# lux-liang/Robust-Audio-Deepfake-Evolution

Measured on AMD Instinct MI355X. Metric: Phase-6 train throughput (utterances/sec), DualStreamSEMamba + LoRA + RawBoost/codec + FGM, higher is better.
Workload: dtype fp16; 1 GPU; Phase6_Proposed.conf train step on ASVspoof19-LA-shaped utterances; micro_batch=8, accumulation=4, global_batch=32, seq_len=64600, parallelism=dp1, fgm=True, mixup=True, rawboost_algo=5, lora_mode=reference, hip_graphs=True, window_batched_clean_passes=True

## Files before the change

### include/radhip.h

```cpp
#ifndef RADHIP_H
#define RADHIP_H

#include <stdint.h>

#ifdef __cplusplus
extern "C" {
#endif

#define RDX_OK 0
#define RDX_EINVAL (-1)
#define RDX_EUNSUPPORTED (-2)

typedef enum { RDX_F32 = 0, RDX_BF16 = 1 } rdx_dtype;

const char* rdx_version(void);
const char* rdx_strerror(int code);

int rdx_sincconv_absmaxpool_fwd(const float* x, int64_t batch, int64_t len, const float* filters,
                                int channels, int ksize, int mask_lo, int mask_hi, float* out,
                                void* stream);
int rdx_sincconv_absmaxpool_fwd_devmask(const float* x, int64_t batch, int64_t len,
                                        const float* filters, int channels, int ksize,
                                        const int32_t* mask_dev, int mask_stride, float* out,
                                        void* stream);
// ... 315 lines not shown
int rdx_adamw_many_max(void);
int rdx_adamw_many(int n, float* const* params, float* const* grads, float* const* exp_avg, float* const* exp_avg_sq,
                   const float* const* step, const int64_t* numel, double lr, double beta1, double beta2,
                   double weight_decay, double eps, const float* grad_scale, const float* found_inf, void* stream);

int rdx_timestamp_acc(int64_t* acc, int sign, void* stream);
int rdx_wallclock_khz(int device);

int rdx_gemm_bf16_strided(const void* A, int64_t lda, int64_t sA, const void* B, int64_t ldb, void* C, int64_t ldc,
                          int64_t crow, int batch, int M, int N, int K, const void* bias, void* stream);

int rdx_fe_conv0(const float* x, int64_t batch, int64_t len, const float* w, const float* bias, const float* gamma,
                 const float* beta, float eps, int ksize, int stride, void* out, void* stream);
int rdx_fe_ln_gelu(void* io, int64_t rows, const float* gamma, const float* beta, float eps, float* out32,
                   void* stream);

int rdx_sconv_fwd(const void* x, const void* w, void* y, void* y2, const float* bn, int N, int H, int W, int ci,
                  int co, int kh, int ph, void* stream);
int rdx_sconv_fwd_res(const void* x, const void* w, void* y, const void* res, int N, int H, int W, int ci, int co,
                      int kh, int ph, void* stream);
int rdx_sconv_dgrad_bnselu(const void* dy, const void* w, const void* c, void* dc, const float* bn, float* sums,
                           int N, int H, int W, int ci, int co, int kh, int ph, void* stream);
int rdx_sconv_fwd_pool(const void* x, const void* w, const void* idn, const float* bias, void* y, uint8_t* arg, int N,
                       int H, int W, int ci, int co, void* stream);
int rdx_sconv_fwd_res_pool(const void* x, const void* w, void* y, const void* dp, const uint8_t* arg, float* dbias,
                           int N, int H, int W, int ci, int co, int kh, int ph, void* stream);
int rdx_sconv_dgrad_bnselu_pool(const void* dp, const uint8_t* arg, const void* w, const void* c, void* dc,
                                const float* bn, float* sums, int N, int H, int W, int ci, int co, int kh, int ph,
                                void* stream);
int rdx_sconv_dgrad_pool(const void* dp, const uint8_t* arg, const void* w, void* dx, int N, int H, int W, int ci,
                         int co, int kh, int ph, void* stream);
int rdx_sconv_wgrad_pool(const void* x, const void* dp, const uint8_t* arg, float* dw, float* part, int N, int H,
                         int W, int ci, int co, int kh, int ph, void* stream);
int rdx_sconv_wgrad_nblk(int N, int Ho, int W);
int rdx_sconv_wgrad(const void* x, const void* dy, float* dw, float* part, int N, int H, int W, int ci, int co,
                    int kh, int ph, void* stream);
int rdx_se_fwd(const void* x, const void* w1, const void* w2, void* y, void* m, void* h, void* s, int B, int T, int C,
               int R, void* stream);
int64_t rdx_se_bwd_part_floats(int B, int C, int R);
int rdx_se_bwd(const void* dy, const void* x, const void* w1, const void* w2, const void* m, const void* h, const void* s,
               void* dx, float* part, float* dw1, float* dw2, int B, int T, int C, int R, void* stream);
int rdx_attn_pool_fwd(const void* f, const void* w, const void* bias, void* feat, float* a, int B, int T, int C,
                      void* stream);
int rdx_attn_pool_bwd(const void* f, const void* w, const float* a, const void* dfeat, void* df, float* part, float* dw,
                      float* db, int B, int T, int C, void* stream);
int rdx_upcat_fwd(const void* fw, const void* fs, void* out, int B, int T1, int T2, int C, void* stream);
int rdx_upcat_bwd(const void* dout, void* dfs, int B, int T1, int T2, int C, void* stream);
int rdx_sconv_wprep_many(int n, const float* const* src, void* const* wf, void* const* wd, const int* co,
                         const int* ci, const int* kh, void* stream);

#ifdef __cplusplus
}
#endif
#endif
```

### robust-audio-deepfake-evolution_amd/csrc/sconv.hip

```cpp
#include <climits>
#include <initializer_list>

#include "common.h"

namespace rdx {

typedef __attribute__((ext_vector_type(16))) float sf32x16;
typedef __attribute__((ext_vector_type(2))) unsigned int v2u32;

constexpr int SC_T = 256;
constexpr int SC_P = 128;
constexpr int SC_PW = SC_P + 2;

__device__ __forceinline__ sf32x16 sc_mfma(hx8 a, hx8 b, sf32x16 c) {
  return mfma32x32x16(a, b, c);
}
__device__ __forceinline__ uint32_t sc_pack2(float a, float b) {
  hst x = f2h(a), y = f2h(b);
  return (uint32_t)(*reinterpret_cast<uint16_t*>(&x)) | ((uint32_t)(*reinterpret_cast<uint16_t*>(&y)) << 16);
}
__device__ __forceinline__ float sc_selu(float u) {
  return 1.0507009873554805f * (u > 0.f ? u : 1.6732632423543772f * (__expf(u) - 1.0f));
}

template <int C>
__device__ __forceinline__ int sc_off(int row, int ch) {
  constexpr int NCH = C / 8;
  return row * (C * 2) + 16 * (ch ^ (row & (NCH - 1)));
}

struct SConvArgs {
  const hst* x;
  const hst* w;
  hst* y;
  hst* y2;
  const float* bn;
  const hst* c;
  float* sums;
  const hst* res;
  const uint8_t* xarg;
  const uint8_t* rarg;
  uint8_t* parg;
  int N, H, W, Ho, ph;
  int rows_per;
};

constexpr uint32_t SC_OOB = 0x80000000u;

__device__ __forceinline__ __amdgpu_buffer_rsrc_t sc_rsrc(const void* p, int64_t bytes) {
  return __builtin_amdgcn_make_buffer_rsrc(const_cast<void*>(p), 0, (int)bytes, 0x00020000);
}

template <int CI, int PW = SC_PW>
__device__ __forceinline__ void sc_load_row(uint4* regs, __amdgpu_buffer_rsrc_t rs, int hi, int H, int W, int p0) {
  constexpr int XCH = CI / 8, NV = (PW * XCH + SC_T - 1) / SC_T;
  const bool rok = hi >= 0 && hi < H;
#pragma unroll
  for (int j = 0; j < NV; ++j) {
    const int i = threadIdx.x + SC_T * j;
    const int ch = i % XCH, pp = i / XCH, wi = p0 - 1 + pp;
    const bool ok = rok && pp < PW && wi >= 0 && wi < W;
    const uint32_t off = ok ? (uint32_t)(((hi * W + wi) * CI + ch * 8) * 2) : SC_OOB;
    regs[j] = __builtin_bit_cast(uint4, __builtin_amdgcn_raw_buffer_load_b128(rs, off, 0, 0));
  }
}
template <int CI, int PW = SC_PW>
__device__ __forceinline__ void sc_store_row(char* slot, const uint4* regs) {
  constexpr int XCH = CI / 8, NV = (PW * XCH + SC_T - 1) / SC_T;
#pragma unroll
  for (int j = 0; j < NV; ++j) {
    const int i = threadIdx.x + SC_T * j;
    if (i < PW * XCH) *reinterpret_cast<uint4*>(slot + sc_off<CI>(i / XCH, i % XCH)) = regs[j];
  }
}

__device__ __forceinline__ uint32_t sc_exp2(uint32_t d, uint32_t ab, uint32_t j) {
  return d & (((ab & 0xffu) == j ? 0xffffu : 0u) | (((ab >> 8) & 0xffu) == j ? 0xffff0000u : 0u));
}
__device__ __forceinline__ uint4 sc_expand(uint4 d, uint2 ab, uint32_t j) {
  return make_uint4(sc_exp2(d.x, ab.x, j), sc_exp2(d.y, ab.x >> 16, j), sc_exp2(d.z, ab.y, j),
                    sc_exp2(d.w, ab.y >> 16, j));
}

template <int CI>
__device__ __forceinline__ void sc_load_row_exp(uint4* regs, uint2* aregs, __amdgpu_buffer_rsrc_t rs,
                                                __amdgpu_buffer_rsrc_t ra, int hi, int H, int Wo, int p0) {
  constexpr int XCH = CI / 8, NV = (SC_PW * XCH + SC_T - 1) / SC_T;
  const bool rok = hi >= 0 && hi < H;
#pragma unroll
  for (int j = 0; j < NV; ++j) {
    const int i = threadIdx.x + SC_T * j;
    const int ch = i % XCH, pp = i / XCH, wi = p0 - 1 + pp;
    const int wo = wi / 3;
    const bool ok = rok && pp < SC_PW && wi >= 0 && wo < Wo;
    const uint32_t e = (uint32_t)((hi * Wo + wo) * CI + ch * 8);
    regs[j] = __builtin_bit_cast(uint4, __builtin_amdgcn_raw_buffer_load_b128(rs, ok ? e * 2 : SC_OOB, 0, 0));
    aregs[j] = __builtin_bit_cast(uint2, __builtin_amdgcn_raw_buffer_load_b64(ra, ok ? e : SC_OOB, 0, 0));
  }
}
template <int CI>
__device__ __forceinline__ void sc_store_row_exp(char* slot, const uint4* regs, const uint2* aregs, int p0) {
  constexpr int XCH = CI / 8, NV = (SC_PW * XCH + SC_T - 1) / SC_T;
#pragma unroll
  for (int j = 0; j < NV; ++j) {
// ... 242 lines not shown
    __syncthreads();
  }
  if constexpr (NSUM > 0) {
#pragma unroll
    for (int q = 0; q < NSUM; ++q)
#pragma unroll
      for (int t = 0; t < NT; ++t)
#pragma unroll
        for (int g = 0; g < 4; ++g)
#pragma unroll
          for (int e = 0; e < 4; ++e) {
            float x = bsum[q][t][g][e];
#pragma unroll
            for (int o = 1; o < 32; o <<= 1) x += __shfl_xor(x, o, 64);
            bsum[q][t][g][e] = x;
          }
    float* red = reinterpret_cast<float*>(sc_lds);
    if (r == 0) {
#pragma unroll
      for (int q = 0; q < NSUM; ++q)
#pragma unroll
        for (int t = 0; t < NT; ++t)
#pragma unroll
          for (int g = 0; g < 4; ++g)
#pragma unroll
            for (int e = 0; e < 4; ++e) red[(wv * NSUM + q) * CO + t * 32 + 8 * g + 4 * h + e] = bsum[q][t][g][e];
    }
    __syncthreads();
    for (int i = tid; i < NSUM * CO; i += SC_T)
      atomicAdd(&a.sums[i], (red[i] + red[NSUM * CO + i]) + (red[2 * NSUM * CO + i] + red[3 * NSUM * CO + i]));
  }
}

struct SWgradArgs {
  const hst* x;
  const hst* dy;
  const uint8_t* arg;
  float* part;
  int N, H, W, Ho, ph;
  int64_t units;
  int strips, nz, rows_per;
};


template <int C>
__device__ __forceinline__ int sc_img(int row, int ch) {
  return (C * 16) * (row >> 3) + 512 * (ch >> 2) + 64 * (row & 7) + 16 * ((ch & 3) ^ ((row >> 2) & 3));
}
template <int C>
__device__ __forceinline__ hx8 sc_read_tr(const char* img, int r0, int c0, int s, int lane) {
  const int g = lane >> 4, i = lane & 15;
  const int row = r0 + 16 * s + 4 * (g >> 1) + (i >> 2);
  const int col = c0 + 16 * (g & 1) + 4 * (i & 3);
  const int sub = 2 * (col & 7);
  const hx4v lo = ds_tr4((img + sc_img<C>(row, col >> 3) + sub));
  const hx4v hi = ds_tr4((img + sc_img<C>(row + 8, col >> 3) + sub));
  hx8 r;
#pragma unroll
  for (int j = 0; j < 4; ++j) {
    r[j] = lo[j];
    r[4 + j] = hi[j];
  }
  return r;
}

constexpr int SC_XR = 136;
// ... 134 lines not shown
  sconv_wgrad_body<CI, CO, KH, true>(a);
}

constexpr int SC_RS = 16;
__global__ void sconv_wgrad_reduce1_kernel(const float* __restrict__ part, int nblk, int64_t n, float* __restrict__ part2) {
  const int64_t i = (int64_t)blockIdx.x * blockDim.x + threadIdx.x;
  if (i >= n) return;
  const int per = (nblk + SC_RS - 1) / SC_RS, b0 = blockIdx.y * per, b1 = min(nblk, b0 + per);
  float s[8] = {0.f, 0.f, 0.f, 0.f, 0.f, 0.f, 0.f, 0.f};
  int b = b0;
  for (; b + 8 <= b1; b += 8) {
#pragma unroll
    for (int k = 0; k < 8; ++k) s[k] += part[(int64_t)(b + k) * n + i];
  }
  for (; b < b1; ++b) s[0] += part[(int64_t)b * n + i];
  part2[(int64_t)blockIdx.y * n + i] = ((s[0] + s[1]) + (s[2] + s[3])) + ((s[4] + s[5]) + (s[6] + s[7]));
}
__global__ void sconv_wgrad_reduce2_kernel(const float* __restrict__ part2, int64_t n, float* __restrict__ dw) {
  const int64_t i = (int64_t)blockIdx.x * blockDim.x + threadIdx.x;
  if (i >= n) return;
  float s = 0.f;
#pragma unroll
  for (int z = 0; z < SC_RS; ++z) s += part2[(int64_t)z * n + i];
  dw[i] = s;
}

static int sc_per_cu(size_t smem) {
  const int n = (int)((160 * 1024) / smem);
  return n < 1 ? 1 : (n > 4 ? 4 : n);
}

static size_t sc_wgrad_smem(int ci, int co, int kh) { return (2 * (size_t)SC_P * co + (size_t)(kh + 1) * SC_XR * ci) * 2; }

template <int CI, int CO, int KH, bool kBnBwd = false, bool kPool = false, bool kExpIn = false, bool kExpRes = false>
static int sconv_fwd_launch(const SConvArgs& a, hipStream_t st) {
  if ((int64_t)a.H * a.W * CI * 2 >= (int64_t)SC_OOB - 4096 || (int64_t)a.Ho * a.W * CO * 2 >= (int64_t)SC_OOB - 4096)
    return RDX_EUNSUPPORTED;
  if ((kPool || kExpIn || kExpRes) && a.W < 3) return RDX_EUNSUPPORTED;
  const size_t smem = (size_t)(KH + 1) * (kPool ? SC_PPW : SC_PW) * CI * 2 + (size_t)KH * 3 * CO * CI * 2 +
                      5 * CO * sizeof(float);
  const int strips = kPool ? (a.W / 3 * 3 + SC_PP - 1) / SC_PP : (a.W + SC_P - 1) / SC_P;
  const int64_t slots = 256 * (int64_t)sc_per_cu(smem), pairs = (int64_t)strips * a.N;
  int nz = 1;
  int64_t best = -1;
  for (int z = 1; z <= a.Ho && z <= 64; ++z) {
    const int rp = (a.Ho + z - 1) / z;
    if (z > 1 && (a.Ho + rp - 1) / rp < z) continue;
    const int64_t cost = ((pairs * z + slots - 1) / slots) * (rp + KH + 1);
    if (best < 0 || cost < best) {
      best = cost;
      nz = z;
    }
  }
  SConvArgs b = a;
  b.rows_per = (a.Ho + nz - 1) / nz;
  dim3 grid((unsigned)strips, (unsigned)a.N, (unsigned)((a.Ho + b.rows_per - 1) / b.rows_per));
  hipLaunchKernelGGL((sconv_fwd_kernel<CI, CO, KH, kBnBwd, kPool, kExpIn, kExpRes>), grid, dim3(SC_T), smem, st, b);
  RDX_LAUNCH_CHECK();
  return RDX_OK;
}

template <int CI, int CO, int KH, bool kExp = false>
static int sconv_wgrad_launch(const SWgradArgs& a, int nblk, hipStream_t st) {
  const size_t smem = sc_wgrad_smem(CI, CO, KH);
  if constexpr (kExp)
    hipLaunchKernelGGL((sconv_wgrad_pool_kernel<CI, CO, KH>), dim3((unsigned)nblk), dim3(SC_T), smem, st, a);
  else
    hipLaunchKernelGGL((sconv_wgrad_kernel<CI, CO, KH>), dim3((unsigned)nblk), dim3(SC_T), smem, st, a);
  RDX_LAUNCH_CHECK();
  return RDX_OK;
}

}

using namespace rdx;

#define SC_ALL(X, ...)                                                                                         \
  X(32, 32, 2, __VA_ARGS__) X(32, 64, 2, __VA_ARGS__) X(64, 32, 2, __VA_ARGS__) X(64, 64, 2, __VA_ARGS__)      \
  X(32, 64, 1, __VA_ARGS__) X(64, 32, 1, __VA_ARGS__) X(32, 32, 1, __VA_ARGS__) X(64, 64, 1, __VA_ARGS__)
#define SC_SQUARE(X, ...) X(32, 32, 2, __VA_ARGS__) X(64, 64, 2, __VA_ARGS__)
#define SC_DOWN_DGRAD(X, ...) X(64, 32, 1, __VA_ARGS__)
#define SC_DOWN_WGRAD(X, ...) X(32, 64, 1, __VA_ARGS__)
#define SC_HAS(CI, CO, KH, ...) || (ci == CI && co == CO && kh == KH)
#define SC_CONV(CI, CO, KH, ...) \
  if (ci == CI && co == CO && kh == KH) return sconv_fwd_launch<CI, CO, KH, __VA_ARGS__>(a, as_stream(stream));
#define SC_WGRAD(CI, CO, KH, ...) \
  if (ci == CI && co == CO && kh == KH) return sconv_wgrad_launch<CI, CO, KH, __VA_ARGS__>(a, nblk, st);

static bool sc_square(int ci, int co, int kh) { return false SC_SQUARE(SC_HAS, 0); }

static bool sc_ptrs_ok(std::initializer_list<const void*> ps) {
  for (const void* p : ps)
    if (!p || ((uintptr_t)p & 15) != 0) return false;
  return true;
}

static bool sc_geom_ok(int N, int H, int W, int kh, int ph, int max_n = 65535) {
  return N > 0 && N <= max_n && H > 0 && W > 0 && ph >= 0 && ph <= kh;
}

static SConvArgs sc_args(const void* x, const void* w, void* y, int N, int H, int W, int kh, int ph) {
  SConvArgs a{};
  a.x = (const hst*)x;
  a.w = (const hst*)w;
  a.y = (hst*)y;
  a.N = N;
  a.H = H;
  a.W = W;
  a.ph = ph;
  a.Ho = H + 2 * ph - kh + 1;
  return a;
}

extern "C" int rdx_sconv_fwd(const void* x, const void* w, void* y, void* y2, const float* bn, int N, int H, int W,
                             int ci, int co, int kh, int ph, void* stream) {
  RDX_REQUIRE(sc_ptrs_ok({x, w, y}) && (!y2 || (sc_ptrs_ok({y2}) && bn)));
  RDX_REQUIRE(sc_geom_ok(N, H, W, kh, ph) && (kh == 1 || kh == 2));
  SConvArgs a = sc_args(x, w, y, N, H, W, kh, ph);
  RDX_REQUIRE(a.Ho > 0);
  a.y2 = (hst*)y2;
  a.bn = bn;
  SC_ALL(SC_CONV, false)
  return RDX_EUNSUPPORTED;
}

extern "C" int rdx_sconv_fwd_res(const void* x, const void* w, void* y, const void* res, int N, int H, int W, int ci,
                                 int co, int kh, int ph, void* stream) {
  RDX_REQUIRE(sc_ptrs_ok({x, w, y, res}) && sc_geom_ok(N, H, W, kh, ph) && (kh == 1 || kh == 2));
  SConvArgs a = sc_args(x, w, y, N, H, W, kh, ph);
  RDX_REQUIRE(a.Ho > 0);
  a.res = (const hst*)res;
  SC_ALL(SC_CONV, false)
  return RDX_EUNSUPPORTED;
}

extern "C" int rdx_sconv_dgrad_bnselu(const void* dy, const void* w, const void* c, void* dc, const float* bn,
                                      float* sums, int N, int H, int W, int ci, int co, int kh, int ph, void* stream) {
  RDX_REQUIRE(sc_ptrs_ok({dy, w, c, dc}) && bn && sums && sc_geom_ok(N, H, W, kh, ph));
  if (!sc_square(ci, co, kh)) return RDX_EUNSUPPORTED;
  SConvArgs a = sc_args(dy, w, dc, N, H, W, kh, ph);
  RDX_REQUIRE(a.Ho > 0);
  a.bn = bn;
  a.c = (const hst*)c;
  a.sums = sums;
  SC_SQUARE(SC_CONV, true)
  return RDX_EUNSUPPORTED;
}

extern "C" int rdx_sconv_fwd_pool(const void* x, const void* w, const void* idn, const float* bias, void* y,
                                  uint8_t* arg, int N, int H, int W, int ci, int co, void* stream) {
  const int kh = 2;
  RDX_REQUIRE(sc_ptrs_ok({x, w, idn, y, arg}) && bias && sc_geom_ok(N, H, W, kh, 0) && H > 1);
  if (!sc_square(ci, co, kh) || W < 3) return RDX_EUNSUPPORTED;
  SConvArgs a = sc_args(x, w, y, N, H, W, kh, 0);
  a.bn = bias;
  a.res = (const hst*)idn;
  a.parg = arg;
  SC_SQUARE(SC_CONV, false, true)
  return RDX_EUNSUPPORTED;
}

extern "C" int rdx_sconv_fwd_res_pool(const void* x, const void* w, void* y, const void* dp, const uint8_t* arg,
                                      float* dbias, int N, int H, int W, int ci, int co, int kh, int ph, void* stream) {
  RDX_REQUIRE(sc_ptrs_ok({x, w, y, dp, arg}) && dbias && sc_geom_ok(N, H, W, kh, ph) && (kh == 1 || kh == 2));
  SConvArgs a = sc_args(x, w, y, N, H, W, kh, ph);
  RDX_REQUIRE(a.Ho > 0);
  a.sums = dbias;
  a.res = (const hst*)dp;
  a.rarg = arg;
  SC_SQUARE(SC_CONV, false, false, false, true)
  return RDX_EUNSUPPORTED;
}

extern "C" int rdx_sconv_dgrad_bnselu_pool(const void* dp, const uint8_t* arg, const void* w, const void* c, void* dc,
                                           const float* bn, float* sums, int N, int H, int W, int ci, int co, int kh,
                                           int ph, void* stream) {
  RDX_REQUIRE(sc_ptrs_ok({dp, arg, w, c, dc}) && bn && sums && sc_geom_ok(N, H, W, kh, ph));
  if (!sc_square(ci, co, kh) || W < 3) return RDX_EUNSUPPORTED;
  SConvArgs a = sc_args(dp, w, dc, N, H, W, kh, ph);
  RDX_REQUIRE(a.Ho > 0);
  a.bn = bn;
  a.c = (const hst*)c;
  a.sums = sums;
  a.xarg = arg;
  SC_SQUARE(SC_CONV, true, false, true)
  return RDX_EUNSUPPORTED;
}

extern "C" int rdx_sconv_dgrad_pool(const void* dp, const uint8_t* arg, const void* w, void* dx, int N, int H, int W,
                                    int ci, int co, int kh, int ph, void* stream) {
  RDX_REQUIRE(sc_ptrs_ok({dp, arg, w, dx}) && sc_geom_ok(N, H, W, 1, 0));
  if (ph != 0 || W < 3) return RDX_EUNSUPPORTED;
  SConvArgs a = sc_args(dp, w, dx, N, H, W, 1, 0);
  a.xarg = arg;
  SC_DOWN_DGRAD(SC_CONV, false, false, true)
  return RDX_EUNSUPPORTED;
}

constexpr int SC_WP_MAX = 32;
struct WPrepTable {
  const float* src[SC_WP_MAX];
  hst* wf[SC_WP_MAX];
  hst* wd[SC_WP_MAX];
  int co[SC_WP_MAX], ci[SC_WP_MAX], kh[SC_WP_MAX];
};
__global__ __launch_bounds__(256) void sconv_wprep_many_kernel(WPrepTable t) {
  const int k = blockIdx.y;
  const int co = t.co[k], ci = t.ci[k], kh = t.kh[k];
  const int n = co * ci * kh * 3;
  for (int i = blockIdx.x * 256 + threadIdx.x; i < n; i += gridDim.x * 256) {
    const int kw = i % 3, r = i / 3, h = r % kh, r2 = r / kh, c = r2 % ci, o = r2 / ci;
    const hst v = f2h(t.src[k][i]);
    t.wf[k][((int64_t)(h * 3 + kw) * co + o) * ci + c] = v;
    t.wd[k][((int64_t)((kh - 1 - h) * 3 + (2 - kw)) * ci + c) * co + o] = v;
  }
}

extern "C" int rdx_sconv_wprep_many(int n, const float* const* src, void* const* wf, void* const* wd, const int* co,
                                    const int* ci, const int* kh, void* stream) {
  RDX_REQUIRE(n >= 0 && (n == 0 || (src && wf && wd && co && ci && kh)));
  if (n > SC_WP_MAX) return RDX_EUNSUPPORTED;
  if (n == 0) return RDX_OK;
  WPrepTable t{};
  int mx = 1;
  for (int k = 0; k < n; ++k) {
    RDX_REQUIRE(src[k] && wf[k] && wd[k] && co[k] > 0 && ci[k] > 0 && (kh[k] == 1 || kh[k] == 2));
    t.src[k] = src[k];
    t.wf[k] = reinterpret_cast<hst*>(wf[k]);
    t.wd[k] = reinterpret_cast<hst*>(wd[k]);
// ... 84 lines not shown
```

### robust-audio-deepfake-evolution_amd/radhip/_lib.py

```python
import ctypes
import os
import threading

_HERE = os.path.dirname(os.path.abspath(__file__))
LIB_PATH = os.environ.get("RADHIP_LIB", os.path.join(_HERE, "libradhip.so"))
LIB16_PATH = os.environ.get("RADHIP_LIB16", os.path.join(_HERE, "libradhip_f16.so"))

RDX_F32 = 0
RDX_BF16 = 1
EPI_BIAS, EPI_BIAS_GELU, EPI_GELU_BWD, EPI_RESID_DROP = 0, 1, 2, 3
EPI_F32, EPI_F32_GELU_SPLIT = 4, 5

c_int = ctypes.c_int
c_i64 = ctypes.c_int64
c_f32 = ctypes.c_float
c_f64 = ctypes.c_double
c_vp = ctypes.c_void_p
c_fp = ctypes.c_void_p


class RawboostUtt(ctypes.Structure):

    _fields_ = [
        ("offset", c_i64),
# ... 121 lines not shown
    "rdx_sincconv_absmaxpool_f16mfma": (c_int, [c_vp, c_i64, c_i64, c_vp, c_int, c_int, c_int, c_int, c_vp, c_int,
                                                c_vp, c_vp]),
    "rdx_scan2_chunks": (c_int, [c_int]),
    "rdx_scan2_rec_elems": (c_i64, [c_int, c_int, c_int, c_int, c_int]),
    "rdx_scan2_fwd": (c_int, [c_int] + [c_vp] * 5 + [c_i64] + [c_vp] * 6 + [c_int] * 5 + [c_vp]),
    "rdx_scan2_bwd": (c_int, [c_int] + [c_vp] * 5 + [c_i64] + [c_vp] * 5 + [c_i64] + [c_vp] * 6 + [c_i64, c_vp]
                      + [c_int] * 5 + [c_vp]),
    "rdx_pgemm_bf16": (c_int, [c_vp, c_i64, c_vp, c_i64, c_vp, c_i64, c_int, c_int, c_int, c_vp, c_int, c_vp, c_i64,
                               c_vp, c_i64, c_int, c_int, c_vp]),
    "rdx_pgemm_prof": (c_int, [c_vp, c_i64, c_vp, c_i64, c_vp, c_i64, c_int, c_int, c_int, c_vp, c_int, c_int, c_vp,
                               c_vp]),
    "rdx_hgemm": (c_int, [c_vp, c_i64, c_vp, c_i64, c_vp, c_i64, c_int, c_int, c_int, c_vp, c_int, c_vp, c_i64, c_vp,
                          c_i64, c_int, c_int, c_int, c_vp, c_i64, c_vp, c_i64, c_vp]),
    "rdx_hgemm_ws_bytes": (c_i64, [c_int, c_int, c_int, c_int]),
    "rdx_colsum_many": (c_int, [c_int, c_vp, c_vp, c_vp, c_vp, c_vp, c_vp]),
    "rdx_lgemm": (c_int, [c_vp, c_i64, c_int, c_vp, c_i64, c_vp, c_i64, c_int, c_int, c_int, c_int, c_vp, c_int,
                          c_vp, c_i64, c_vp, c_i64, c_vp, c_i64, c_vp]),
    "rdx_hgemm_counters": (c_i64, [c_int, c_int, c_int]),
    "rdx_hgemm_sk_ws_bytes": (c_i64, [c_int, c_int, c_int, c_int]),
    "rdx_gemm_bf16_strided": (c_int, [c_vp, c_i64, c_i64, c_vp, c_i64, c_vp, c_i64, c_i64, c_int, c_int, c_int, c_int,
                                      c_vp, c_vp]),
    "rdx_fe_conv0": (c_int, [c_vp, c_i64, c_i64, c_vp, c_vp, c_vp, c_vp, c_f32, c_int, c_int, c_vp, c_vp]),
    "rdx_fe_ln_gelu": (c_int, [c_vp, c_i64, c_vp, c_vp, c_f32, c_vp, c_vp]),
    "rdx_sconv_dgrad_bnselu": (c_int, [c_vp, c_vp, c_vp, c_vp, c_vp, c_vp, c_int, c_int, c_int, c_int, c_int, c_int,
                                       c_int, c_vp]),
    "rdx_sconv_fwd": (c_int, [c_vp, c_vp, c_vp, c_vp, c_vp, c_int, c_int, c_int, c_int, c_int, c_int, c_int, c_vp]),
    "rdx_sconv_fwd_res": (c_int, [c_vp, c_vp, c_vp, c_vp, c_int, c_int, c_int, c_int, c_int, c_int, c_int, c_vp]),
    "rdx_sconv_fwd_pool": (c_int, [c_vp] * 6 + [c_int] * 5 + [c_vp]),
    "rdx_sconv_fwd_res_pool": (c_int, [c_vp] * 6 + [c_int] * 7 + [c_vp]),
    "rdx_sconv_dgrad_bnselu_pool": (c_int, [c_vp] * 7 + [c_int] * 7 + [c_vp]),
    "rdx_sconv_dgrad_pool": (c_int, [c_vp] * 4 + [c_int] * 7 + [c_vp]),
    "rdx_sconv_wgrad_pool": (c_int, [c_vp] * 5 + [c_int] * 7 + [c_vp]),
    "rdx_sconv_wgrad_nblk": (c_int, [c_int, c_int, c_int]),
    "rdx_sconv_wgrad": (c_int, [c_vp, c_vp, c_vp, c_vp, c_int, c_int, c_int, c_int, c_int, c_int, c_int, c_vp]),
    "rdx_sconv_wprep_many": (c_int, [c_int, c_vp, c_vp, c_vp, c_vp, c_vp, c_vp, c_vp]),
    "rdx_se_fwd": (c_int, [c_vp] * 7 + [c_int] * 4 + [c_vp]),
    "rdx_se_bwd_part_floats": (c_i64, [c_int, c_int, c_int]),
    "rdx_se_bwd": (c_int, [c_vp] * 11 + [c_int] * 4 + [c_vp]),
    "rdx_attn_pool_fwd": (c_int, [c_vp] * 5 + [c_int] * 3 + [c_vp]),
    "rdx_attn_pool_bwd": (c_int, [c_vp] * 8 + [c_int] * 3 + [c_vp]),
    "rdx_upcat_fwd": (c_int, [c_vp] * 3 + [c_int] * 4 + [c_vp]),
    "rdx_upcat_bwd": (c_int, [c_vp] * 2 + [c_int] * 4 + [c_vp]),
    "rdx_attn_fwd": (c_int, [c_vp, c_i64, c_vp, c_i64, c_vp, c_i64, c_vp, c_vp, c_vp, c_int, c_f32, c_f32, c_vp, c_i64,
                             c_vp, c_vp, c_int, c_int, c_int, c_int, c_vp]),
    "rdx_attn_keep_mask_words": (c_i64, [c_int, c_int, c_int]),
    "rdx_attn_bwd": (c_int, [c_vp, c_i64, c_vp, c_i64, c_vp, c_i64, c_vp, c_vp, c_vp, c_int, c_f32, c_f32, c_vp, c_i64,
                             c_vp, c_vp, c_i64, c_vp, c_vp, c_vp, c_vp, c_i64, c_vp, c_int, c_int, c_int, c_int, c_vp]),
    "rdx_attn_bwd_fused": (c_int, [c_vp, c_i64, c_vp, c_i64, c_vp, c_i64, c_vp, c_vp, c_vp, c_f32, c_f32, c_vp, c_i64,
                                   c_vp, c_vp, c_i64, c_vp, c_vp, c_vp, c_vp, c_i64, c_vp, c_int, c_int, c_int, c_int,
                                   c_vp]),
    "rdx_attn_bwd_split_ws": (c_i64, [c_int, c_int]),
    "rdx_attn_bwd_fused_split": (c_int, [c_vp, c_i64, c_vp, c_i64, c_vp, c_i64, c_vp, c_vp, c_vp, c_f32, c_f32, c_vp,
                                         c_i64, c_vp, c_vp, c_i64, c_vp, c_vp, c_vp, c_vp, c_i64, c_vp, c_vp, c_i64,
                                         c_vp, c_i64, c_int, c_int, c_int, c_int, c_vp]),
    "rdx_attn_dropout_mask": (c_int, [c_vp, c_int, c_f32, c_vp, c_i64, c_int, c_vp]),
    "rdx_dropout_mask": (c_int, [c_vp, c_int, c_f32, c_vp, c_i64, c_vp]),
    "rdx_wl_ln1_fwd": (c_int, [c_vp] * 3 + [c_f32] + [c_vp] * 5 + [c_int, c_vp,
                       c_int, c_int, c_f32, c_vp, c_i64] + [c_vp] * 3
                       + [c_i64, c_int, c_vp]),
    "rdx_wl_add_ln_fwd": (c_int, [c_vp, c_vp, c_vp, c_int, c_f32, c_vp, c_vp,
                          c_vp, c_f32, c_vp, c_vp, c_vp, c_i64, c_int,
                          c_vp]),
    "rdx_wl_residual": (c_int, [c_vp, c_vp, c_vp, c_int, c_f32, c_vp, c_i64,
                        c_vp]),
    "rdx_wl_dropout_bwd": (c_int, [c_vp, c_vp, c_int, c_f32, c_vp, c_i64,
                           c_vp]),
# ... 103 lines not shown
```

### robust-audio-deepfake-evolution_amd/radhip/ops.py

```python
import ctypes
import os

import numpy as np
import torch

from . import _lib
from ._lib import check, lib, ptr_array

HALF = (torch.bfloat16, torch.float16)
_DT = {torch.float32: _lib.RDX_F32, torch.bfloat16: _lib.RDX_BF16, torch.float16: _lib.RDX_BF16}


def _L(*xs):
    dts = {x if isinstance(x, torch.dtype) else x.dtype for x in xs}
    if torch.float16 in dts:
        if torch.bfloat16 in dts:
            raise TypeError("radhip: one launch cannot mix bf16 and fp16 tensors")
        return _lib.lib16()
    return lib()


def half_dtype():
    if torch.is_autocast_enabled("cuda"):
        d = torch.get_autocast_dtype("cuda")
# ... 1081 lines not shown

class Block0Convs(torch.autograd.Function):

    @staticmethod
    def forward(ctx, x, w1, wd):
        _require_gpu(x)
        hd = half_dtype()
        xb = x.to(hd)
        w1b, wdb = w1.to(hd), wd.to(hd)
        c = torch.nn.functional.conv2d(xb, w1b, None, 1, (1, 1))
        idn = torch.nn.functional.conv2d(xb, wdb, None, 1, (0, 1))
        ctx.save_for_backward(xb, w1b, wdb)
        ctx.meta = (w1.shape, wd.shape, x.dtype)
        return c, idn

    @staticmethod
    def backward(ctx, dc, di):
        xb, w1b, wdb = ctx.saved_tensors
        w1_shape, wd_shape, x_dtype = ctx.meta
        dc = _nhwc(dc.to(xb.dtype))
        di = _nhwc(di.to(xb.dtype))
        xc = xb.contiguous(memory_format=torch.channels_last)
        dx, dw1, dwd = _b0_bwd(xc, dc, di, w1b.float().contiguous(), wdb.float().contiguous(), (w1_shape, wd_shape))
        return dx.to(x_dtype), dw1, dwd


SCONV_CH = (32, 64)


def sconv_enabled():
    return os.environ.get("RADHIP_SCONV", "1") != "0"


def sconv_weight_ok(weight):
    co, ci, kh, kw = weight.shape
    return ci in SCONV_CH and co in SCONV_CH and kh in (1, 2) and kw == 3 and sconv_enabled()


def sconv_ok(x, weight):
    return x.is_cuda and x.dim() == 4 and x.shape[1] == weight.shape[1] and sconv_weight_ok(weight)


SCONV_WCACHE = None


def _sconv_w(weight, hd):
    if SCONV_WCACHE is not None:
        hit = SCONV_WCACHE.get((id(weight), hd))
        if hit is not None and hit[0] is weight:
            return hit[1], hit[2]
    wf, wd = _sconv_w_prep(weight, hd)
    if SCONV_WCACHE is not None:
        SCONV_WCACHE[(id(weight), hd)] = (weight, wf, wd)
    return wf, wd


def _sconv_w_prep(weight, hd):
    co, ci, kh, kw = weight.shape
    wb = weight.detach().to(hd)
    wf = wb.permute(2, 3, 0, 1).reshape(kh * kw, co, ci).contiguous()
    wd = wb.flip(2, 3).permute(2, 3, 1, 0).reshape(kh * kw, ci, co).contiguous()
    return wf, wd


def sconv_prep_many(weights, hd):
    cache = SCONV_WCACHE
    ws = [w for w in weights if w.is_cuda and w.dtype == torch.float32 and w.is_contiguous() and sconv_weight_ok(w)]
    if cache is None or not ws:
        return
    for i in range(0, len(ws), 32):
        g = ws[i:i + 32]
        wf, wd = [], []
        for w in g:
            co, ci, kh, kw = w.shape
            wf.append(torch.empty(kh * kw, co, ci, device=w.device, dtype=hd))
            wd.append(torch.empty(kh * kw, ci, co, device=w.device, dtype=hd))
        n = len(g)
        ints = lambda vals: (ctypes.c_int * n)(*vals)
        check(_L(hd).rdx_sconv_wprep_many(n, ptr_array([w.data_ptr() for w in g]), ptr_array([t.data_ptr() for t in wf]),
                                          ptr_array([t.data_ptr() for t in wd]), ints([w.shape[0] for w in g]),
                                          ints([w.shape[1] for w in g]), ints([w.shape[2] for w in g]),
                                          _stream(g[0])), "sconv_wprep_many")
        for w, a, b in zip(g, wf, wd):
            cache[(id(w), hd)] = (w, a, b)


def _sconv_run(x, w_tap, ci, co, kh, ph, y2=None, bn=None, res=None):
    N, _, H, W = x.shape
    Ho = H + 2 * ph - kh + 1
    y = _empty_nhwc((N, co, Ho, W), x)
    nbytes = 2.0 * (N * H * W * ci + N * Ho * W * co * (2 if (y2 is not None or res is not None) else 1))
    with _timed("sconv_fwd", x, nbytes, shape=(N, H, W, ci, co, kh, ph)):
        if res is not None:
            if res.shape != y.shape or res.dtype != y.dtype or not res.is_contiguous(memory_format=torch.channels_last):
                raise ValueError("radhip sconv: residual must be NHWC of the output's shape and dtype")
            check(_L(x).rdx_sconv_fwd_res(_p(x), _p(w_tap), _p(y), _p(res), N, H, W, ci, co, kh, ph, _stream(x)),
                  "sconv_fwd_res")
        else:
            check(_L(x).rdx_sconv_fwd(_p(x), _p(w_tap), _p(y), _p(y2) if y2 is not None else None,
                                      _p(bn) if bn is not None else None, N, H, W, ci, co, kh, ph, _stream(x)),
                  "sconv_fwd")
    return y


SCONV_POOL_DEFAULT = "1"


def sconv_pool_ok(w2_shape, W, half):
    co, ci, kh, kw = w2_shape
    return (ci == co and ci in SCONV_CH and kh == 2 and kw == 3 and W >= 3
            and os.environ.get("RADHIP_SCONV_POOL", SCONV_POOL_DEFAULT) in ("1", half))


def _sconv_run_pool(x, w_tap, idn, bias, c):
    N, _, H, W = x.shape
    Ho = H - 1
    if idn.shape != (N, c, Ho, W) or idn.dtype != x.dtype or not idn.is_contiguous(memory_format=torch.channels_last):
        raise ValueError("radhip sconv: identity must be NHWC of the convolution output's shape and dtype")
    y = _empty_nhwc((N, c, Ho, W // 3), x)
    arg = _empty_nhwc((N, c, Ho, W // 3), x, torch.uint8)
    nbytes = 2.0 * (N * H * W * c + N * Ho * W * c) + 3.0 * y.numel()
    with _timed("sconv_fwd", x, nbytes, shape=(N, H, W, c, c, 2, 0)):
        check(_L(x).rdx_sconv_fwd_pool(_p(x), _p(w_tap), _p(idn), _p(bias), _p(y), _p(arg), N, H, W, c, c, _stream(x)),
              "sconv_fwd_pool")
    return y, arg


def _sconv_run_res_pool(x, w_tap, dp, arg, dbias, ci, co, kh, ph):
    N, _, H, W = x.shape
    Ho = H + 2 * ph - kh + 1
    y = _empty_nhwc((N, co, Ho, W), x)
    nbytes = 2.0 * (N * H * W * ci + N * Ho * W * co) + 3.0 * dp.numel()
    with _timed("sconv_fwd", x, nbytes, shape=(N, H, W, ci, co, kh, ph)):
        check(_L(x).rdx_sconv_fwd_res_pool(_p(x), _p(w_tap), _p(y), _p(dp), _p(arg), _p(dbias), N, H, W, ci, co, kh, ph,
                                           _stream(x)), "sconv_fwd_res_pool")
    return y


def _sconv_wgrad_pool(x, dp, arg, weight_shape):
    co, ci, kh, kw = weight_shape
    N, _, H, W = x.shape
    Ho = dp.shape[2]
    nblk = lib().rdx_sconv_wgrad_nblk(N, Ho, W)
    part = torch.empty(nblk, kh * 3 * co * ci, device=x.device, dtype=torch.float32)
    dw = torch.empty(kh * 3, co, ci, device=x.device, dtype=torch.float32)
    with _timed("sconv_wgrad", x, 2.0 * N * H * W * ci + 3.0 * dp.numel(), shape=(N, H, W, ci, co, kh, 0)):
        check(_L(x).rdx_sconv_wgrad_pool(_p(x), _p(dp), _p(arg), _p(dw), _p(part), N, H, W, ci, co, kh, 0, _stream(x)),
              "sconv_wgrad_pool")
    return dw.view(kh, 3, co, ci).permute(2, 3, 0, 1)


def _sconv_dgrad_pool(dp, arg, wd, weight_shape, W):
    co, ci, kh, kw = weight_shape
    N, _, H, _ = dp.shape
    dx = _empty_nhwc((N, ci, H, W), dp)
    with _timed("sconv_fwd", dp, 3.0 * dp.numel() + 2.0 * dx.numel(), shape=(N, H, W, co, ci, kh, 0)):
        check(_L(dp).rdx_sconv_dgrad_pool(_p(dp), _p(arg), _p(wd), _p(dx), N, H, W, co, ci, kh, 0, _stream(dp)),
              "sconv_dgrad_pool")
    return dx


def _pooled_grad_ok(dy, arg):
    return dy.shape == arg.shape and dy.data_ptr() % 16 == 0


def _sconv_backward(x, dy, wd, weight_shape, ph, need_dx):
    co, ci, kh, kw = weight_shape
# ... 899 lines not shown
```

Baseline: 518.8 utt/s.

## Add specialized 64-channel 2x3 sconv kernel with register-resident weights and 512 threads

Adds a dedicated kernel for 64-in/64-out 2x3 convolutions that keeps all weight fragments in registers, uses 512-thread blocks split into output-channel halves and strip quarters, and restages outputs through per-wave LDS tiles for coalesced stores. It covers the plain, residual, pool and expanded-residual epilogues. It is dispatched by default through a runtime select flag controlled by an environment variable. The aim is to cut repeated weight LDS traffic and raise MFMA utilization on the dominant conv shape, at the cost of higher register pressure and a second code path to maintain.

After: 519.9 utt/s (median of 5 runs). No clear change (+0.2%).

```diff
diff --git a/include/radhip.h b/include/radhip.h
--- a/include/radhip.h
+++ b/include/radhip.h
@@ -371,6 +371,8 @@
                          int co, int kh, int ph, void* stream);
 int rdx_sconv_wgrad_pool(const void* x, const void* dp, const uint8_t* arg, float* dw, float* part, int N, int H,
                          int W, int ci, int co, int kh, int ph, void* stream);
+int rdx_sconv64_select(int on);
+int rdx_sconv64_rows_per(int N, int Ho, int W, int pool);
 int rdx_sconv_wgrad_nblk(int N, int Ho, int W);
 int rdx_sconv_wgrad(const void* x, const void* dy, float* dw, float* part, int N, int H, int W, int ci, int co,
                     int kh, int ph, void* stream);
diff --git a/robust-audio-deepfake-evolution_amd/csrc/sconv.hip b/robust-audio-deepfake-evolution_amd/csrc/sconv.hip
--- a/robust-audio-deepfake-evolution_amd/csrc/sconv.hip
+++ b/robust-audio-deepfake-evolution_amd/csrc/sconv.hip
@@ -7,6 +7,7 @@
 
 typedef __attribute__((ext_vector_type(16))) float sf32x16;
 typedef __attribute__((ext_vector_type(2))) unsigned int v2u32;
+typedef __attribute__((ext_vector_type(4))) unsigned int v4u32;
 
 constexpr int SC_T = 256;
 constexpr int SC_P = 128;
@@ -51,25 +52,25 @@
   return __builtin_amdgcn_make_buffer_rsrc(const_cast<void*>(p), 0, (int)bytes, 0x00020000);
 }
 
-template <int CI, int PW = SC_PW>
+template <int CI, int PW = SC_PW, int T = SC_T>
 __device__ __forceinline__ void sc_load_row(uint4* regs, __amdgpu_buffer_rsrc_t rs, int hi, int H, int W, int p0) {
-  constexpr int XCH = CI / 8, NV = (PW * XCH + SC_T - 1) / SC_T;
+  constexpr int XCH = CI / 8, NV = (PW * XCH + T - 1) / T;
   const bool rok = hi >= 0 && hi < H;
 #pragma unroll
   for (int j = 0; j < NV; ++j) {
-    const int i = threadIdx.x + SC_T * j;
+    const int i = threadIdx.x + T * j;
     const int ch = i % XCH, pp = i / XCH, wi = p0 - 1 + pp;
     const bool ok = rok && pp < PW && wi >= 0 && wi < W;
     const uint32_t off = ok ? (uint32_t)(((hi * W + wi) * CI + ch * 8) * 2) : SC_OOB;
     regs[j] = __builtin_bit_cast(uint4, __builtin_amdgcn_raw_buffer_load_b128(rs, off, 0, 0));
   }
 }
-template <int CI, int PW = SC_PW>
+template <int CI, int PW = SC_PW, int T = SC_T>
 __device__ __forceinline__ void sc_store_row(char* slot, const uint4* regs) {
-  constexpr int XCH = CI / 8, NV = (PW * XCH + SC_T - 1) / SC_T;
+  constexpr int XCH = CI / 8, NV = (PW * XCH + T - 1) / T;
 #pragma unroll
   for (int j = 0; j < NV; ++j) {
-    const int i = threadIdx.x + SC_T * j;
+    const int i = threadIdx.x + T * j;
     if (i < PW * XCH) *reinterpret_cast<uint4*>(slot + sc_off<CI>(i / XCH, i % XCH)) = regs[j];
   }
 }
@@ -378,6 +379,277 @@
   }
 }
 
+constexpr int SW_T = 512;
+constexpr int SW_TILE = 2048;
+
+__device__ __forceinline__ int sw_off(int row, int ch) { return row * 64 + 16 * (ch ^ ((row >> 2) & 3)); }
+__device__ __forceinline__ void sw_sync() {
+  __builtin_amdgcn_fence(__ATOMIC_ACQ_REL, "wavefront");
+  __builtin_amdgcn_wave_barrier();
+}
+
+__device__ __forceinline__ float sw_f32(float x) {
+  asm("" : "+v"(x));
+  return x;
+}
+
+template <int KH, bool kPool = false, bool kExpRes = false>
+__global__ __launch_bounds__(SW_T) void sconv64_kernel(SConvArgs a) {
+  static_assert(!(kPool && kExpRes), "one epilogue at a time");
+  extern __shared__ __attribute__((aligned(16))) char sc_lds[];
+  constexpr int CI = 64, CO = 64;
+  constexpr int PW = kPool ? SC_PPW : SC_PW, PSTEP = kPool ? 30 : 32;
+  constexpr int NSLOT = KH + 1, SLOT = PW * CI * 2, XCH = CI / 8;
+  constexpr int NV = (PW * XCH + SW_T - 1) / SW_T;
+  char* xs = sc_lds;
+  float* sbn = reinterpret_cast<float*>(xs + NSLOT * SLOT);
+  const int tid = threadIdx.x, wv = tid >> 6, lane = tid & 63, r = lane & 31, h = lane >> 5;
+  const int pq = wv & 3, th = wv >> 2;
+  char* tile = reinterpret_cast<char*>(sbn + 5 * CO) + wv * SW_TILE;
+  const int n = blockIdx.y, p0 = kPool ? (int)blockIdx.x * SC_PP - 1 : (int)blockIdx.x * SC_P;
+  const int ho0 = blockIdx.z * a.rows_per, ho1 = min(a.Ho, ho0 + a.rows_per);
+  const int Wo = a.W / 3;
+  const int64_t iel = (int64_t)a.H * a.W * CI, ibytes = iel * 2;
+  const int64_t obytes = (int64_t)a.Ho * a.W * CO * 2, pel = (int64_t)a.Ho * Wo * CO;
+  const int64_t obase_n = (int64_t)n * a.Ho * a.W * CO;
+  const __amdgpu_buffer_rsrc_t rx = sc_rsrc(a.x + (int64_t)n * iel, ibytes);
+  const __amdgpu_buffer_rsrc_t ry =
+      kPool ? sc_rsrc(a.y + (int64_t)n * pel, pel * 2) : sc_rsrc(a.y + obase_n, obytes);
+  const __amdgpu_buffer_rsrc_t rpa = sc_rsrc(kPool ? a.parg + (int64_t)n * pel : (uint8_t*)a.y, kPool ? pel : 0);
+  const __amdgpu_buffer_rsrc_t ry2 = sc_rsrc(a.y2 ? a.y2 + obase_n : a.y + obase_n, a.y2 ? obytes : 0);
+  constexpr bool rexp = kExpRes;
+  const __amdgpu_buffer_rsrc_t rres = rexp      ? sc_rsrc(a.res + (int64_t)n * pel, pel * 2)
+                                      : a.res   ? sc_rsrc(a.res + obase_n, obytes)
+                                                : sc_rsrc(a.y, 0);
+  const __amdgpu_buffer_rsrc_t rra = sc_rsrc(rexp ? a.rarg + (int64_t)n * pel : (const uint8_t*)a.y, rexp ? pel : 0);
+  constexpr int SPK = CI / 16, NSTEP = KH * 3 * SPK, PD = 4;
+  hx8 wq[NSTEP];
+  {
+    const __amdgpu_buffer_rsrc_t rw = sc_rsrc(a.w, (int64_t)KH * 3 * CO * CI * 2);
+#pragma unroll
+    for (int q = 0; q < NSTEP; ++q) {
+      const int tap = q / SPK, s = q % SPK;
+      const uint32_t off = (uint32_t)((((tap * CO + th * 32 + r) * CI) + (2 * s + h) * 8) * 2);
+      wq[q] = __builtin_bit_cast(hx8, __builtin_amdgcn_raw_buffer_load_b128(rw, off, 0, 0));
+    }
+  }
+  if (a.bn && (kPool || a.y2))
+    for (int i = tid; i < (kPool ? 1 : 4) * CO; i += SW_T) sbn[i] = a.bn[i];
+  uint4 pre[NV];
+  auto load_in = [&](int hi) { sc_load_row<CI, PW, SW_T>(pre, rx, hi, a.H, a.W, p0); };
+  auto store_in = [&](char* slot) { sc_store_row<CI, PW, SW_T>(slot, pre); };
+#pragma unroll
+  for (int kh = 0; kh < KH; ++kh) {
+    load_in(ho0 + kh - a.ph);
+    store_in(xs + ((ho0 + kh) % NSLOT) * SLOT);
+  }
+  __syncthreads();
+  const int pw = pq * PSTEP + r;
+  const int p = p0 + pw;
+  const bool pv = p >= 0 && p < a.W;
+  const int rwo = p / 3, rj = p - 3 * rwo;
+  int ppos[2];
+  bool ppv[2];
+#pragma unroll
+  for (int j = 0; j < 2; ++j) {
+    ppos[j] = p0 + pq * PSTEP + ((lane + 64 * j) >> 2);
+    ppv[j] = ppos[j] >= 0 && ppos[j] < a.W;
+  }
+  const int pch = lane & 3;
+  constexpr int NSUM = kExpRes ? 1 : 0;
+  float bsum[NSUM ? NSUM : 1][4][4];
+  if constexpr (NSUM > 0) {
+#pragma unroll
+    for (int q = 0; q < NSUM; ++q)
+#pragma unroll
+      for (int g = 0; g < 4; ++g)
+#pragma unroll
+        for (int e = 0; e < 4; ++e) bsum[q][g][e] = 0.f;
+  }
+  for (int ho = ho0; ho < ho1; ++ho) {
+    const bool more = ho + 1 < ho1;
+    load_in(more ? ho - a.ph + KH : -1);
+    uint32_t poff[2];
+#pragma unroll
+    for (int j = 0; j < 2; ++j)
+      poff[j] = ppv[j] ? (uint32_t)(((ho * a.W + ppos[j]) * CO + th * 32 + pch * 8) * 2) : SC_OOB;
+    const bool side = kPool || (!rexp && a.res);
+    uint4 sin[2];
+    uint2 cres[4];
+    uint32_t cra[4];
+    if constexpr (rexp) {
+      const uint32_t erow = pv && rwo < Wo ? (uint32_t)((ho * Wo + rwo) * CO + th * 32 + 4 * h) : SC_OOB / 2;
+#pragma unroll
+      for (int g = 0; g < 4; ++g) {
+        cres[g] = __builtin_bit_cast(uint2, __builtin_amdgcn_raw_buffer_load_b64(rres, (erow + 8 * g) * 2, 0, 0));
+        cra[g] = __builtin_amdgcn_raw_buffer_load_b32(rra, erow + 8 * g, 0, 0);
+      }
+    } else if (side) {
+#pragma unroll
+      for (int j = 0; j < 2; ++j)
+        sin[j] = __builtin_bit_cast(uint4, __builtin_amdgcn_raw_buffer_load_b128(rres, poff[j], 0, 0));
+    }
+    sf32x16 acc;
+#pragma unroll
+    for (int i = 0; i < 16; ++i) acc[i] = 0.f;
+    const char* xk0 = xs + (ho % NSLOT) * SLOT;
+    const char* xk1 = xs + ((ho + 1) % NSLOT) * SLOT;
+    hx8 xq[NSTEP];
+#pragma unroll
+    for (int q = 0; q < NSTEP + PD; ++q) {
+      if (q < NSTEP) {
+        const int kh = q / (3 * SPK), kw = (q / SPK) % 3, s = q % SPK;
+        xq[q] = *reinterpret_cast<const hx8*>((kh ? xk1 : xk0) + sc_off<CI>(pw + kw, 2 * s + h));
+      }
+      if (q >= PD) acc = sc_mfma(wq[q - PD], xq[q - PD], acc);
+      __builtin_amdgcn_sched_barrier(0);
+    }
+    if (more) store_in(xs + ((ho + KH) % NSLOT) * SLOT);
+    if constexpr (!rexp) {
+      if (side) {
+        sw_sync();
+#pragma unroll
+        for (int j = 0; j < 2; ++j)
+          *reinterpret_cast<uint4*>(tile + sw_off((lane + 64 * j) >> 2, pch)) = sin[j];
+        sw_sync();
+#pragma unroll
+        for (int g = 0; g < 4; ++g) cres[g] = *reinterpret_cast<const uint2*>(tile + sw_off(r, g) + 8 * h);
+      }
+    }
+    uint2 vo[4], uo[4];
+    uint32_t bo[4];
+#pragma unroll
+    for (int g = 0; g < 4; ++g) {
+      const int co = th * 32 + 8 * g + 4 * h;
+      float v[4];
+#pragma unroll
+      for (int e = 0; e < 4; ++e) v[e] = acc[4 * g + e];
+      if constexpr (kPool) {
+        const uint2 ii = cres[g];
+        const float iv[4] = {hlo(ii.x), hhi(ii.x), hlo(ii.y), hhi(ii.y)};
+        const float4 bq = *reinterpret_cast<const float4*>(sbn + co);
+        const float pb[4] = {bq.x, bq.y, bq.z, bq.w};
+        float best[4];
+        uint32_t bi = 0;
+#pragma unroll
+        for (int e = 0; e < 4; ++e) {
+          const float s0 = hround(v[e]) + iv[e] + pb[e];
+          const float s1 = dpp_f32<0x101>(s0);
+          const float s2 = dpp_f32<0x102>(s0);
+          float b = s0;
+          uint32_t k = 0;
+          if (s1 > b || s1 != s1) {
+            b = s1;
+            k = 1;
+          }
+          if (s2 > b || s2 != s2) {
+            b = s2;
+            k = 2;
+          }
+          best[e] = b;
+          bi |= k << (8 * e);
+        }
+        vo[g] = make_uint2(sc_pack2(best[0], best[1]), sc_pack2(best[2], best[3]));
+        bo[g] = bi;
+        continue;
+      }
+      if (a.res) {
+        uint2 rr = cres[g];
+        if constexpr (rexp) {
+          rr.x = sc_exp2(rr.x, cra[g], (uint32_t)rj);
+          rr.y = sc_exp2(rr.y, cra[g] >> 16, (uint32_t)rj);
+          bsum[0][g][0] += hlo(rr.x);
+          bsum[0][g][1] += hhi(rr.x);
+          bsum[0][g][2] += hlo(rr.y);
+          bsum[0][g][3] += hhi(rr.y);
+        }
+        v[0] = hround(v[0]) + hlo(rr.x);
+        v[1] = hround(v[1]) + hhi(rr.x);
+        v[2] = hround(v[2]) + hlo(rr.y);
+        v[3] = hround(v[3]) + hhi(rr.y);
+      }
+      vo[g] = make_uint2(sc_pack2(v[0], v[1]), sc_pack2(v[2], v[3]));
+      if (a.y2) {
+        const float4 cb = *reinterpret_cast<const float4*>(sbn + co);
+        const float4 mu = *reinterpret_cast<const float4*>(sbn + CO + co);
+        const float4 sg = *reinterpret_cast<const float4*>(sbn + 2 * CO + co);
+        const float4 bb = *reinterpret_cast<const float4*>(sbn + 3 * CO + co);
+        const float pcb[4] = {cb.x, cb.y, cb.z, cb.w}, pmu[4] = {mu.x, mu.y, mu.z, mu.w};
+        const float psg[4] = {sg.x, sg.y, sg.z, sg.w}, pbb[4] = {bb.x, bb.y, bb.z, bb.w};
+        float u[4];
+#pragma unroll
+        for (int e = 0; e < 4; ++e)
+          u[e] = sw_f32(sc_selu(fmaf((hround(v[e]) + pcb[e]) - pmu[e], psg[e], pbb[e])));
+        uo[g] = make_uint2(sc_pack2(u[0], u[1]), sc_pack2(u[2], u[3]));
+      }
+    }
+    sw_sync();
+    if constexpr (kPool) {
+      if (r % 3 == 1 && r < 30) {
+        const int k = r / 3;
+#pragma unroll
+        for (int g = 0; g < 4; ++g) {
+          *reinterpret_cast<uint2*>(tile + sw_off(k, g) + 8 * h) = vo[g];
+          *reinterpret_cast<uint32_t*>(tile + 1024 + k * 32 + 8 * g + 4 * h) = bo[g];
+        }
+      }
+      sw_sync();
+      const int k = lane >> 2, wo = (int)blockIdx.x * (SC_PP / 3) + pq * 10 + k;
+      const uint32_t e = lane < 40 && wo < Wo ? (uint32_t)((ho * Wo + wo) * CO + th * 32 + pch * 8) : SC_OOB / 2;
+      const uint4 q = *reinterpret_cast<const uint4*>(tile + sw_off(k, pch));
+      const uint2 b = *reinterpret_cast<const uint2*>(tile + 1024 + lane * 8);
+      __builtin_amdgcn_raw_buffer_store_b128(__builtin_bit_cast(v4u32, q), ry, e * 2, 0, 0);
+      __builtin_amdgcn_raw_buffer_store_b64(__builtin_bit_cast(v2u32, b), rpa, e, 0, 0);
+    } else {
+#pragma unroll
+      for (int g = 0; g < 4; ++g) *reinterpret_cast<uint2*>(tile + sw_off(r, g) + 8 * h) = vo[g];
+      sw_sync();
+#pragma unroll
+      for (int j = 0; j < 2; ++j) {
+        const uint4 q = *reinterpret_cast<const uint4*>(tile + sw_off((lane + 64 * j) >> 2, pch));
+        __builtin_amdgcn_raw_buffer_store_b128(__builtin_bit_cast(v4u32, q), ry, poff[j], 0, 0);
+      }
+      if (a.y2) {
+        sw_sync();
+#pragma unroll
+        for (int g = 0; g < 4; ++g) *reinterpret_cast<uint2*>(tile + sw_off(r, g) + 8 * h) = uo[g];
+        sw_sync();
+#pragma unroll
+        for (int j = 0; j < 2; ++j) {
+          const uint4 q = *reinterpret_cast<const uint4*>(tile + sw_off((lane + 64 * j) >> 2, pch));
+          __builtin_amdgcn_raw_buffer_store_b128(__builtin_bit_cast(v4u32, q), ry2, poff[j], 0, 0);
+        }
+      }
+    }
+    __syncthreads();
+  }
+  if constexpr (NSUM > 0) {
+#pragma unroll
+    for (int q = 0; q < NSUM; ++q)
+#pragma unroll
+      for (int g = 0; g < 4; ++g)
+#pragma unroll
+        for (int e = 0; e < 4; ++e) {
+          float x = bsum[q][g][e];
+#pragma unroll
+          for (int o = 1; o < 32; o <<= 1) x += __shfl_xor(x, o, 64);
+          bsum[q][g][e] = x;
+        }
+    float* red = reinterpret_cast<float*>(sc_lds);
+    if (r == 0) {
+#pragma unroll
+      for (int q = 0; q < NSUM; ++q)
+#pragma unroll
+        for (int g = 0; g < 4; ++g)
+#pragma unroll
+          for (int e = 0; e < 4; ++e) red[(pq * NSUM + q) * CO + th * 32 + 8 * g + 4 * h + e] = bsum[q][g][e];
+    }
+    __syncthreads();
+    for (int i = tid; i < NSUM * CO; i += SW_T)
+      atomicAdd(&a.sums[i], (red[i] + red[NSUM * CO + i]) + (red[2 * NSUM * CO + i] + red[3 * NSUM * CO + i]));
+  }
+}
+
 struct SWgradArgs {
   const hst* x;
   const hst* dy;
@@ -578,6 +850,21 @@
 
 static size_t sc_wgrad_smem(int ci, int co, int kh) { return (2 * (size_t)SC_P * co + (size_t)(kh + 1) * SC_XR * ci) * 2; }
 
+static int sc_rows_per(int64_t pairs, int64_t slots, int Ho, int KH) {
+  int nz = 1;
+  int64_t best = -1;
+  for (int z = 1; z <= Ho && z <= 64; ++z) {
+    const int rp = (Ho + z - 1) / z;
+    if (z > 1 && (Ho + rp - 1) / rp < z) continue;
+    const int64_t cost = ((pairs * z + slots - 1) / slots) * (rp + KH + 1);
+    if (best < 0 || cost < best) {
+      best = cost;
+      nz = z;
+    }
+  }
+  return (Ho + nz - 1) / nz;
+}
+
 template <int CI, int CO, int KH, bool kBnBwd = false, bool kPool = false, bool kExpIn = false, bool kExpRes = false>
 static int sconv_fwd_launch(const SConvArgs& a, hipStream_t st) {
   if ((int64_t)a.H * a.W * CI * 2 >= (int64_t)SC_OOB - 4096 || (int64_t)a.Ho * a.W * CO * 2 >= (int64_t)SC_OOB - 4096)
@@ -587,21 +874,33 @@
                       5 * CO * sizeof(float);
   const int strips = kPool ? (a.W / 3 * 3 + SC_PP - 1) / SC_PP : (a.W + SC_P - 1) / SC_P;
   const int64_t slots = 256 * (int64_t)sc_per_cu(smem), pairs = (int64_t)strips * a.N;
-  int nz = 1;
-  int64_t best = -1;
-  for (int z = 1; z <= a.Ho && z <= 64; ++z) {
-    const int rp = (a.Ho + z - 1) / z;
-    if (z > 1 && (a.Ho + rp - 1) / rp < z) continue;
-    const int64_t cost = ((pairs * z + slots - 1) / slots) * (rp + KH + 1);
-    if (best < 0 || cost < best) {
-      best = cost;
-      nz = z;
-    }
-  }
   SConvArgs b = a;
-  b.rows_per = (a.Ho + nz - 1) / nz;
+  b.rows_per = sc_rows_per(pairs, slots, a.Ho, KH);
   dim3 grid((unsigned)strips, (unsigned)a.N, (unsigned)((a.Ho + b.rows_per - 1) / b.rows_per));
   hipLaunchKernelGGL((sconv_fwd_kernel<CI, CO, KH, kBnBwd, kPool, kExpIn, kExpRes>), grid, dim3(SC_T), smem, st, b);
+  RDX_LAUNCH_CHECK();
+  return RDX_OK;
+}
+
+static int sc64_on = 1;
+static bool sc64(int ci, int co, int kh) { return sc64_on && ci == 64 && co == 64 && kh == 2; }
+static int sc64_strips(int W, bool pool) { return pool ? (W / 3 * 3 + SC_PP - 1) / SC_PP : (W + SC_P - 1) / SC_P; }
+static int sc64_rows_per(int N, int Ho, int W, bool pool) {
+  return sc_rows_per((int64_t)sc64_strips(W, pool) * N, 256, Ho, 2);
+}
+
+template <int KH, bool kPool = false, bool kExpRes = false>
+static int sconv64_launch(const SConvArgs& a, hipStream_t st) {
+  static_assert(KH == 2, "the 2 x 3 convolutions");
+  if ((int64_t)a.H * a.W * 64 * 2 >= (int64_t)SC_OOB - 4096 || (int64_t)a.Ho * a.W * 64 * 2 >= (int64_t)SC_OOB - 4096)
+    return RDX_EUNSUPPORTED;
+  if ((kPool || kExpRes) && a.W < 3) return RDX_EUNSUPPORTED;
+  const size_t smem = (size_t)(KH + 1) * (kPool ? SC_PPW : SC_PW) * 64 * 2 + 5 * 64 * sizeof(float) +
+                      (size_t)(SW_T / 64) * SW_TILE;
+  SConvArgs b = a;
+  b.rows_per = sc64_rows_per(a.N, a.Ho, a.W, kPool);
+  dim3 grid((unsigned)sc64_strips(a.W, kPool), (unsigned)a.N, (unsigned)((a.Ho + b.rows_per - 1) / b.rows_per));
+  hipLaunchKernelGGL((sconv64_kernel<KH, kPool, kExpRes>), grid, dim3(SW_T), smem, st, b);
   RDX_LAUNCH_CHECK();
   return RDX_OK;
 }
@@ -666,6 +965,7 @@
   RDX_REQUIRE(a.Ho > 0);
   a.y2 = (hst*)y2;
   a.bn = bn;
+  if (sc64(ci, co, kh)) return sconv64_launch<2>(a, as_stream(stream));
   SC_ALL(SC_CONV, false)
   return RDX_EUNSUPPORTED;
 }
@@ -676,6 +976,7 @@
   SConvArgs a = sc_args(x, w, y, N, H, W, kh, ph);
   RDX_REQUIRE(a.Ho > 0);
   a.res = (const hst*)res;
+  if (sc64(ci, co, kh)) return sconv64_launch<2>(a, as_stream(stream));
   SC_ALL(SC_CONV, false)
   return RDX_EUNSUPPORTED;
 }
@@ -702,6 +1003,7 @@
   a.bn = bias;
   a.res = (const hst*)idn;
   a.parg = arg;
+  if (sc64(ci, co, kh)) return sconv64_launch<2, true>(a, as_stream(stream));
   SC_SQUARE(SC_CONV, false, true)
   return RDX_EUNSUPPORTED;
 }
@@ -714,6 +1016,7 @@
   a.sums = dbias;
   a.res = (const hst*)dp;
   a.rarg = arg;
+  if (sc64(ci, co, kh)) return sconv64_launch<2, false, true>(a, as_stream(stream));
   SC_SQUARE(SC_CONV, false, false, false, true)
   return RDX_EUNSUPPORTED;
 }
@@ -741,6 +1044,16 @@
   a.xarg = arg;
   SC_DOWN_DGRAD(SC_CONV, false, false, true)
   return RDX_EUNSUPPORTED;
+}
+
+extern "C" int rdx_sconv64_select(int on) {
+  sc64_on = on != 0;
+  return RDX_OK;
+}
+
+extern "C" int rdx_sconv64_rows_per(int N, int Ho, int W, int pool) {
+  if (N <= 0 || Ho <= 0 || W <= 0) return RDX_EINVAL;
+  return sc64_rows_per(N, Ho, W, pool != 0);
 }
 
 constexpr int SC_WP_MAX = 32;
diff --git a/robust-audio-deepfake-evolution_amd/radhip/_lib.py b/robust-audio-deepfake-evolution_amd/radhip/_lib.py
--- a/robust-audio-deepfake-evolution_amd/radhip/_lib.py
+++ b/robust-audio-deepfake-evolution_amd/radhip/_lib.py
@@ -177,6 +177,8 @@
     "rdx_sconv_dgrad_pool": (c_int, [c_vp] * 4 + [c_int] * 7 + [c_vp]),
     "rdx_sconv_wgrad_pool": (c_int, [c_vp] * 5 + [c_int] * 7 + [c_vp]),
     "rdx_sconv_wgrad_nblk": (c_int, [c_int, c_int, c_int]),
+    "rdx_sconv64_select": (c_int, [c_int]),
+    "rdx_sconv64_rows_per": (c_int, [c_int, c_int, c_int, c_int]),
     "rdx_sconv_wgrad": (c_int, [c_vp, c_vp, c_vp, c_vp, c_int, c_int, c_int, c_int, c_int, c_int, c_int, c_vp]),
     "rdx_sconv_wprep_many": (c_int, [c_int, c_vp, c_vp, c_vp, c_vp, c_vp, c_vp, c_vp]),
     "rdx_se_fwd": (c_int, [c_vp] * 7 + [c_int] * 4 + [c_vp]),
diff --git a/robust-audio-deepfake-evolution_amd/radhip/ops.py b/robust-audio-deepfake-evolution_amd/radhip/ops.py
--- a/robust-audio-deepfake-evolution_amd/radhip/ops.py
+++ b/robust-audio-deepfake-evolution_amd/radhip/ops.py
@@ -1137,6 +1137,16 @@
     return os.environ.get("RADHIP_SCONV", "1") != "0"
 
 
+def sconv64_enabled():
+    return os.environ.get("RADHIP_SCONV64", "1") != "0"
+
+
+def _sconv_lib(x):
+    L = _L(x)
+    L.rdx_sconv64_select(1 if sconv64_enabled() else 0)
+    return L
+
+
 def sconv_weight_ok(weight):
     co, ci, kh, kw = weight.shape
     return ci in SCONV_CH and co in SCONV_CH and kh in (1, 2) and kw == 3 and sconv_enabled()
@@ -1199,10 +1209,10 @@
         if res is not None:
             if res.shape != y.shape or res.dtype != y.dtype or not res.is_contiguous(memory_format=torch.channels_last):
                 raise ValueError("radhip sconv: residual must be NHWC of the output's shape and dtype")
-            check(_L(x).rdx_sconv_fwd_res(_p(x), _p(w_tap), _p(y), _p(res), N, H, W, ci, co, kh, ph, _stream(x)),
+            check(_sconv_lib(x).rdx_sconv_fwd_res(_p(x), _p(w_tap), _p(y), _p(res), N, H, W, ci, co, kh, ph, _stream(x)),
                   "sconv_fwd_res")
         else:
-            check(_L(x).rdx_sconv_fwd(_p(x), _p(w_tap), _p(y), _p(y2) if y2 is not None else None,
+            check(_sconv_lib(x).rdx_sconv_fwd(_p(x), _p(w_tap), _p(y), _p(y2) if y2 is not None else None,
                                       _p(bn) if bn is not None else None, N, H, W, ci, co, kh, ph, _stream(x)),
                   "sconv_fwd")
     return y
@@ -1226,7 +1236,7 @@
     arg = _empty_nhwc((N, c, Ho, W // 3), x, torch.uint8)
     nbytes = 2.0 * (N * H * W * c + N * Ho * W * c) + 3.0 * y.numel()
     with _timed("sconv_fwd", x, nbytes, shape=(N, H, W, c, c, 2, 0)):
-        check(_L(x).rdx_sconv_fwd_pool(_p(x), _p(w_tap), _p(idn), _p(bias), _p(y), _p(arg), N, H, W, c, c, _stream(x)),
+        check(_sconv_lib(x).rdx_sconv_fwd_pool(_p(x), _p(w_tap), _p(idn), _p(bias), _p(y), _p(arg), N, H, W, c, c, _stream(x)),
               "sconv_fwd_pool")
     return y, arg
 
@@ -1237,7 +1247,7 @@
     y = _empty_nhwc((N, co, Ho, W), x)
     nbytes = 2.0 * (N * H * W * ci + N * Ho * W * co) + 3.0 * dp.numel()
     with _timed("sconv_fwd", x, nbytes, shape=(N, H, W, ci, co, kh, ph)):
-        check(_L(x).rdx_sconv_fwd_res_pool(_p(x), _p(w_tap), _p(y), _p(dp), _p(arg), _p(dbias), N, H, W, ci, co, kh, ph,
+        check(_sconv_lib(x).rdx_sconv_fwd_res_pool(_p(x), _p(w_tap), _p(y), _p(dp), _p(arg), _p(dbias), N, H, W, ci, co, kh, ph,
                                            _stream(x)), "sconv_fwd_res_pool")
     return y
 
```
